# Fannovel16/stylish-tts

Hardware: AMD Instinct MI355X
Metric: utterances_per_sec (higher is better)
Workload: dtype f32

## Files before the change

include/stylish_hip.h:

```cpp
#ifndef STYLISH_HIP_H_
#define STYLISH_HIP_H_

#include <stddef.h>
#include <stdint.h>

#ifdef __cplusplus
extern "C" {
#endif

typedef struct stts_ctx stts_ctx;

typedef struct stts_model_dims {
  int32_t n_fft, win_length, hop_length, sample_rate;
  int32_t style_dim, inter_dim;
  int32_t dec_hidden, dec_residual;
  int32_t gen_input, gen_hidden, gen_inter, gen_io_kernel;
  int32_t tokens, te_hidden, te_filter, te_heads, te_layers, te_kernel;
  int32_t style_layers;
  int32_t dur_layers, dur_classes, dur_max;
  int32_t pe_inter;
} stts_model_dims;

const char* stts_last_error(void);
int stts_version(void);
// ... 77 lines not shown
} stts_cfm_dims;
int stts_cfm_finalize(stts_ctx* ctx, const stts_cfm_dims* dims);
size_t stts_cfm_workspace_bytes(const stts_ctx* ctx, int64_t rows, int n_utt);
int stts_cfm_estimator(stts_ctx* ctx, void* stream, int n_utt, const int32_t* seg_off_host, const int32_t* seg_off_dev, const float* x, int ld_x,
                       const float* asr, int ld_asr, const float* f0, const float* n_curve, const int32_t* curve_off_host,
                       const int32_t* curve_off_dev, const float* spk_emb, const float* t, const float* sine_noise, float* out, int ld_out,
                       void* workspace, size_t workspace_bytes);

int stts_to_time_major(void* stream, const float* x_bct, int B, int C, int T, float* y, int ldy);
int stts_to_channel_major(void* stream, const float* x, int ldx, int B, int C, int T, float* y_bct);

int stts_conv_stft_transform(stts_ctx* ctx, void* stream, int n_utt, const int32_t* frame_off_host, const int32_t* frame_off_dev,
                             const float* wave, int hop, float* mag, float* x, float* y, int ld);
int stts_conv_stft_inverse(stts_ctx* ctx, void* stream, int n_utt, const int32_t* frame_off_host, const int32_t* frame_off_dev,
                           const float* mag, const float* x, const float* y, int ld, int hop, float* wave_out, void* ws, size_t ws_bytes);

int stts_profile_begin(void);
int stts_profile_end(void* stream, int* launches, double* total_ms, double* total_flops);
int stts_profile_report(void* stream, char* json, size_t json_capacity);

int stts_op_mrf_block(stts_ctx* ctx, void* stream, const char* prefix, int n_utt, const int32_t* seg_off_host,
                      const int32_t* seg_off_dev, const float* x, int ldx, int channels, int kernel, const float* style, float* y,
                      int ldy, void* ws, size_t ws_bytes);

#ifdef STTS_TEST_OPS
int stts_op_conv1d(void* stream, int n_utt, const int32_t* seg_off_host, const int32_t* seg_off_dev, const float* x, int ldx, int cin,
                   const float* w_host, const float* bias_host, int cout, int k, int dil, int act, float* y, int ldy, int force_tile, int precision);
int stts_op_adain_block(stts_ctx* ctx, void* stream, const char* prefix, int n_utt, const int32_t* seg_off_host,
                        const int32_t* seg_off_dev, const float* x, int ldx, int cin, int cout, const float* style, float* y, int ldy,
                        void* ws, size_t ws_bytes);
int stts_op_attention(void* stream, int n_utt, const int32_t* q_off_host, const int32_t* q_off_dev, const int32_t* k_off_host,
                      const int32_t* k_off_dev, const float* q, const float* k, const float* v, float* o, int heads, int kc,
                      const int32_t* band_centre, int window, int kernel);
int stts_bench_gemm(void* stream, int n_utt, int rows_per_utt, int cin, int cout, int k, int tile, int iters, double* avg_ms, int tune);
#endif

#ifdef __cplusplus
}
#endif
#endif
```

stylish_tts_amd/_lib.py:

```python
from __future__ import annotations

import ctypes as C
import os

_HERE = os.path.dirname(os.path.abspath(__file__))
LIB_PATH = os.path.abspath(os.environ["STTS_LIB"]) if os.environ.get("STTS_LIB") else os.path.join(_HERE, "libstylish_hip.so")


class ModelDims(C.Structure):
    _fields_ = [(n, C.c_int32) for n in (
        "n_fft", "win_length", "hop_length", "sample_rate",
        "style_dim", "inter_dim",
        "dec_hidden", "dec_residual",
        "gen_input", "gen_hidden", "gen_inter", "gen_io_kernel",
        "tokens", "te_hidden", "te_filter", "te_heads", "te_layers", "te_kernel",
        "style_layers",
        "dur_layers", "dur_classes", "dur_max",
        "pe_inter",
    )]


class CfmDims(C.Structure):
    _fields_ = [(n, C.c_int32) for n in ("feat_dim", "asr_dim", "spk_dim", "hidden_dim", "emb_dim", "depth", "enc_blocks", "dec_blocks",
                                         "prev_depth", "post_depth", "head_dim")]
# ... 30 lines not shown
    "stts_har_ld": (_I, [_P]),
    "stts_decoder_forward": (_I, [_P, _P, _I, _P, _P, _P, _I, _P, _P, _P, _P, _I, _P, _SZ]),
    "stts_prior_flow_forward": (_I, [_P, _P, _I, _P, _P, _P, _I, _P, _P, _P, _I, _P, _P, _P, _SZ]),
    "stts_harmonic_stft": (_I, [_P, _P, _I, _P, _P, _P, _P, _P, _I, _P, _P, _P, _I, _P, _SZ]),
    "stts_vocoder_forward": (_I, [_P, _P, _I, _P, _P, _P, _I, _P, _P, _P, _I, _P, _P, _P, _I, _P, _SZ]),
    "stts_frame_path": (_I, [_P, _P, _I, _P, _P, _P, _I, _P, _P, _P, _P, _P, _P, _I, _P, _P, _SZ, _I]),
    "stts_frame_offsets": (_I, [_P, _P, _I, _P, _P, _P, _P, _P, _P]),
    "stts_phoneme_workspace_bytes": (_SZ, [_P, _I64, _I64, _I]),
    "stts_text_encoder_forward": (_I, [_P, _P, _I, _I, _P, _P, _P, _P, _I, _P, _P, _SZ]),
    "stts_text_style_forward": (_I, [_P, _P, _I, _I, _P, _P, _P, _I, _P, _P, _SZ]),
    "stts_duration_forward": (_I, [_P, _P, _I, _P, _P, _P, _P, _P, _P, _P, _P, _P, _SZ]),
    "stts_pitch_energy_forward": (_I, [_P, _P, _I, _P, _P, _P, _P, _P, _P, _I, _P, _P, _P, _P, _P, _P, _SZ, _I]),
    "stts_duration_decode": (_I, [_P, _P, _I, _I, _P]),
    "stts_duration_to_alignment": (_I, [_P, _P, _I, _I, _P]),
    "stts_length_regulate": (_I, [_P, _P, _I, _P, _P, _P, _I64, _I, _P, _I, _I, _P, _I, _P]),
    "stts_set_precision": (_I, [_P, _I]),
    "stts_upsample4": (_I, [_P, _P, _I, _P, _P, _P, _P, _P]),
    "stts_euler_step": (_I, [_P, _P, _P, C.c_float, C.c_int64]),
    "stts_cfm_finalize": (_I, [_P, _P]),
    "stts_cfm_workspace_bytes": (_SZ, [_P, _I64, _I]),
    "stts_cfm_estimator": (_I, [_P, _P, _I, _P, _P, _P, _I, _P, _I, _P, _P, _P, _P, _P, _P, _P, _P, _I, _P, _SZ]),
    "stts_to_time_major": (_I, [_P, _P, _I, _I, _I, _P, _I]),
    "stts_to_channel_major": (_I, [_P, _P, _I, _I, _I, _I, _P]),
    "stts_conv_stft_transform": (_I, [_P, _P, _I, _P, _P, _P, _I, _P, _P, _P, _I]),
    "stts_conv_stft_inverse": (_I, [_P, _P, _I, _P, _P, _P, _P, _P, _I, _I, _P, _P, _SZ]),
    "stts_profile_begin": (_I, []),
    "stts_profile_end": (_I, [_P, C.POINTER(_I), C.POINTER(C.c_double), C.POINTER(C.c_double)]),
    "stts_profile_report": (_I, [_P, C.c_char_p, _SZ]),
    "stts_op_mrf_block": (_I, [_P, _P, C.c_char_p, _I, _P, _P, _P, _I, _I, _I, _P, _P, _I, _P, _SZ]),
}
TEST_SIGNATURES = {
    "stts_bench_gemm": (_I, [_P, _I, _I, _I, _I, _I, _I, _I, C.POINTER(C.c_double), _I]),
    "stts_op_conv1d": (_I, [_P, _I, _P, _P, _P, _I, _I, _P, _P, _I, _I, _I, _I, _P, _I, _I, _I]),
    "stts_op_adain_block": (_I, [_P, _P, C.c_char_p, _I, _P, _P, _P, _I, _I, _I, _P, _P, _I, _P, _SZ]),
    "stts_op_attention": (_I, [_P, _I, _P, _P, _P, _P, _P, _P, _P, _P, _I, _I, _P, _I, _I]),
}

_lib = None


def load() -> C.CDLL:
    global _lib
    if _lib is not None:
        return _lib
    if not os.path.exists(LIB_PATH):
        raise RuntimeError(
            f"{LIB_PATH} not found: build it with `python -c 'import __graft_entry__ as g; g.build()'` "
            "(hipcc --offload-arch=gfx950).  There is no CPU fallback."
        )
    try:
        import torch
    except ImportError:
        pass
    lib = C.CDLL(LIB_PATH)
    for name, (res, args) in SIGNATURES.items():
        fn = getattr(lib, name)
        fn.restype = res
        fn.argtypes = args
    for name, (res, args) in TEST_SIGNATURES.items():
        fn = getattr(lib, name, None)
        if fn is not None:
            fn.restype = res
            fn.argtypes = args
    _lib = lib
    return lib

# ... 5 lines not shown
```

stylish_tts_amd/csrc/gemm.hip.h:

```cpp
#pragma once
#include <type_traits>
#include <mutex>
#include <map>
#include <hip/hip_ext.h>
#include <cmath>
#include <algorithm>
#include <vector>

#include "common.h"

namespace stts {

using f32x16 = __attribute__((ext_vector_type(16))) float;
using f32x4 = __attribute__((ext_vector_type(4))) float;

enum Act { ACT_NONE = 0, ACT_SILU = 1, ACT_GELU = 2, ACT_RELU = 3, ACT_LRELU = 4 };
enum Epi {
  EPI_STORE = 0,
  EPI_GATE = 1,
  EPI_SPLIT_ACC = 2,
  EPI_COUPLE = 3,
  EPI_PRIOR = 4,
};

// ... 83 lines not shown
  u32x2 r;
  if constexpr (PREC == PREC_BF16) {
    typedef __bf16 b2 __attribute__((ext_vector_type(2)));
    typedef float f2 __attribute__((ext_vector_type(2)));
    const f2 lo = {v.x, v.y}, hi = {v.z, v.w};
    r.x = __builtin_bit_cast(unsigned, __builtin_convertvector(lo, b2));
    r.y = __builtin_bit_cast(unsigned, __builtin_convertvector(hi, b2));
  } else {
    typedef _Float16 h2 __attribute__((ext_vector_type(2)));
    typedef float f2 __attribute__((ext_vector_type(2)));
    const f2 lo = {v.x, v.y}, hi = {v.z, v.w};
    r.x = __builtin_bit_cast(unsigned, __builtin_convertvector(lo, h2));
    r.y = __builtin_bit_cast(unsigned, __builtin_convertvector(hi, h2));
  }
  return r;
}
__device__ __forceinline__ void split3_bf16(const f32x4 v, u32x2& p0, u32x2& p1, u32x2& p2) {
  typedef __bf16 b2 __attribute__((ext_vector_type(2)));
  typedef float f2 __attribute__((ext_vector_type(2)));
  auto pk = [](float a, float b) { const f2 t = {a, b}; return __builtin_bit_cast(unsigned, __builtin_convertvector(t, b2)); };
  auto lo = [](unsigned u) { return __uint_as_float(u << 16); };
  auto hi = [](unsigned u) { return __uint_as_float(u & 0xffff0000u); };
  p0.x = pk(v.x, v.y); p0.y = pk(v.z, v.w);
  const float r0 = v.x - lo(p0.x), r1 = v.y - hi(p0.x), r2 = v.z - lo(p0.y), r3 = v.w - hi(p0.y);
  p1.x = pk(r0, r1); p1.y = pk(r2, r3);
  p2.x = pk(r0 - lo(p1.x), r1 - hi(p1.x)); p2.y = pk(r2 - lo(p1.y), r3 - hi(p1.y));
}
template <int PREC>
__device__ __forceinline__ f32x16 mfma16(const f32x4 a, const f32x4 b, const f32x16 c) {
  if constexpr (PREC == PREC_BF16 || PREC == PREC_X3) return __builtin_amdgcn_mfma_f32_32x32x16_bf16(__builtin_bit_cast(bf16x8, a), __builtin_bit_cast(bf16x8, b), c, 0, 0, 0);
  else return __builtin_amdgcn_mfma_f32_32x32x16_f16(__builtin_bit_cast(f16x8, a), __builtin_bit_cast(f16x8, b), c, 0, 0, 0);
}

template <int BM, int BN, int WARPS_M, int WARPS_N, int EPI, int KSPLIT = 1, bool GLDS = false, int PREC = PREC_F32, int XAFF = 0, bool MSEG = true,
          bool X16 = false>
__global__ void __launch_bounds__(WARPS_M* WARPS_N * 64 * KSPLIT) conv_gemm_f32(const GemmArgs a) {
  static_assert(!(XAFF && GLDS), "the input affine lives on the register staging path");
  static_assert(!X16 || (PREC != PREC_F32 && !XAFF && EPI == EPI_STORE), "16-bit activation rows: 16-bit operand modes, store epilogue");
  constexpr int NT = WARPS_M * WARPS_N * 64 * KSPLIT;
  constexpr bool B16 = PREC != PREC_F32;
  constexpr bool X3 = PREC == PREC_X3;
  constexpr int NPL = X3 ? 3 : 1;
  static_assert(!X3 || !GLDS || X16, "split fp32: fp32 activation rows are split on the register staging path; LDS-DMA needs pre-split planes");
  static_assert(!(B16 && GLDS) || X16, "LDS-DMA staging of 16-bit operands needs 16-bit activation rows (nothing converts on the way)");
  static_assert(KSPLIT == 1 || KSPLIT == 2, "KSPLIT");
  constexpr int WR = BN / WARPS_N, WC = BM / WARPS_M;
  constexpr int TR = WR / 32, TC = WC / 32;
  constexpr int XL = X16 ? (BN * 4 * NPL + NT - 1) / NT : BN * 8 / NT;
  constexpr int WL = B16 ? (BM * 4 * NPL + NT - 1) / NT : BM * 8 / NT;
  static_assert(WR % 32 == 0 && WC % 32 == 0, "wave tile must be a multiple of 32x32");
  static_assert((X16 || (BN * 8) % NT == 0) && (B16 || (BM * 8) % NT == 0), "tile loads must divide over the block");
  static_assert(EPI == EPI_STORE || EPI == EPI_SPLIT_ACC || TC % 2 == 0, "paired epilogues need an even TC");
  constexpr int NSTAGE = (B16 && GLDS) ? (X3 ? 3 : ((BM + BN) <= 256 ? 8 : 3)) : 2;
  constexpr int SLOTS = X3 ? 12 : ((B16 && KSPLIT == 1) ? 4 : 8);
  constexpr int PLANE = (BN + BM) * 4;
  constexpr int STG16 = PLANE * NPL;
  __shared__ f32x4 lds[NSTAGE * (BN + BM) * SLOTS];

  int bx = blockIdx.x, by = blockIdx.y, bz = blockIdx.z;
  {
    unsigned gy = gridDim.y;
    if (a.capacity) {
      const int lane_ = threadIdx.x & 63;
      int tot = 0;
      for (int u0 = 0; u0 < a.n_utt; u0 += 64) {
        const int u = u0 + lane_;
        tot += u < a.n_utt ? (a.seg_off[u + 1] - a.seg_off[u] + BN - 1) / BN : 0;
      }
#pragma unroll
      for (int o = 32; o > 0; o >>= 1) tot += __shfl_xor(tot, o, 64);
      gy = (unsigned)__builtin_amdgcn_readfirstlane(tot);
      if ((unsigned)by >= gy) return;
    }
    const unsigned gx = gridDim.x, nwg = gx * gy * gridDim.z;
    const unsigned orig = bx + gx * (by + gy * bz);
    const unsigned q = nwg >> 3, r = nwg & 7, xcd = orig & 7;
    const unsigned id = (xcd < r ? xcd * (q + 1) : r * (q + 1) + (xcd - r) * q) + (orig >> 3);
    bx = id % gx;
    by = (id / gx) % gy;
    bz = id / (gx * gy);
  }
  const int ksplit = a.ksplit > 1 ? a.ksplit : 1;
  int utt, ks;
  if (a.compact) {
    ks = bz;
    const int t = by + a.tile0, lane_ = threadIdx.x & 63;
    utt = a.n_utt - 1;
    int base = 0, local = 0;
    bool done = false;
    if (a.uniform_len > 0) {
      const int tpu = (a.uniform_len + BN - 1) / BN;
      utt = t / tpu;
      local = t - utt * tpu;
      done = utt < a.n_utt;
    }
    for (int u0 = 0; u0 < a.n_utt && !done && a.uniform_len <= 0; u0 += 64) {
      const int u = u0 + lane_;
      const int tiles = u < a.n_utt ? (a.seg_off[u + 1] - a.seg_off[u] + BN - 1) / BN : 0;
      int incl = tiles;
#pragma unroll
      for (int d = 1; d < 64; d <<= 1) {
        const int v = __shfl_up(incl, d, 64);
        if (lane_ >= d) incl += v;
      }
      const int excl = incl - tiles;
      const unsigned long long hit = __ballot(t >= base + excl && t < base + incl);
      if (hit) {
        const int src = __ffsll((long long)hit) - 1;
        utt = u0 + src;
        local = t - base - __shfl(excl, src, 64);
        done = true;
      }
      base += __shfl(incl, 63, 64);
    }
    if (!done) return;
    utt = __builtin_amdgcn_readfirstlane(utt);
    by = __builtin_amdgcn_readfirstlane(local);
  } else {
    utt = bz / ksplit;
    ks = bz % ksplit;
  }
  const int lo = a.uniform_len > 0 ? a.uniform_lo0 + utt * a.uniform_len : a.seg_off[utt];
  const int hi = a.uniform_len > 0 ? lo + a.uniform_len : a.seg_off[utt + 1];
  const int row0 = lo + by * BN;
  if (row0 >= hi) return;
  const int m0 = bx * BM;
  const int tid = threadIdx.x, lane = tid & 63;
#ifdef STTS_GEMM_TRACE
  const unsigned dbg_blk = blockIdx.x + gridDim.x * (blockIdx.y + gridDim.y * blockIdx.z);
  auto stamp = [&](int i) { if (a.dbg && tid == 0) a.dbg[8 * (long)dbg_blk + i] = wall_clock64(); };
  const long long dbg_c0 = clock64();
  if (a.dbg && tid == 0) { a.dbg[8 * (long)dbg_blk + 5] = __builtin_amdgcn_s_getreg(0xF804); a.dbg[8 * (long)dbg_blk + 6] = __builtin_amdgcn_s_getreg(0xF814); }
  auto stamp_end = [&]() { stamp(3); if (a.dbg && tid == 0) a.dbg[8 * (long)dbg_blk + 7] = clock64() - dbg_c0; };
  auto ablate = [&](int bit) { return (a.tune & bit) != 0; };
#else
  auto stamp = [&](int) {};
  auto stamp_end = [&]() {};
  auto ablate = [](int) { return false; };
#endif
  stamp(0);
  const int kg = (tid >> 6) / (WARPS_M * WARPS_N), wid = (tid >> 6) % (WARPS_M * WARPS_N);
  const int wn = wid / WARPS_M, wm = wid % WARPS_M;
  (void)kg;

  f32x16 acc[TR][TC];
#pragma unroll
  for (int i = 0; i < TR; ++i)
#pragma unroll
    for (int j = 0; j < TC; ++j)
#pragma unroll
      for (int r = 0; r < 16; ++r) acc[i][j][r] = 0.0f;

  int s = 0, tap = 0, chunk = 0;
  auto xbase = [&](const GemmSeg& g) {
// ... 812 lines not shown
  for (int i = 0; i < a.nseg; ++i) k += (double)a.seg[i].kreal * a.seg[i].ntaps;
  return 2.0 * (double)a.rows_total * (double)a.wrows * k;
}

#define STTS_LAUNCH_TIMED(kernel, grid, block, st, e0, e1, ...)                                   \
  do {                                                                                            \
    if (e0) hipExtLaunchKernelGGL(kernel, grid, block, 0, st, e0, e1, 0, __VA_ARGS__);            \
    else hipLaunchKernelGGL(kernel, grid, block, 0, st, __VA_ARGS__);                             \
  } while (0)

#define STTS_LAUNCH_PROF(name, bytes, kernel, grid, block, st, ...)                                \
  do {                                                                                            \
    stts::GemmProfiler& _p = stts::gemm_profiler();                                               \
    if (_p.on) {                                                                                  \
      hipEvent_t _e0 = _p.next(), _e1 = _p.next();                                                \
      _p.add(name, 1, 0.0, 0.0, (double)(bytes));                                                 \
      hipExtLaunchKernelGGL(kernel, grid, block, 0, st, _e0, _e1, 0, __VA_ARGS__);                \
    } else {                                                                                      \
      hipLaunchKernelGGL(kernel, grid, block, 0, st, __VA_ARGS__);                                \
    }                                                                                             \
  } while (0)

inline bool gemm16_eligible(const GemmArgs& a, int epi, int npad);
inline long gemm16_tiles(const GemmArgs& a, int npad, int n_utt);
inline bool gemm16_will_run(const GemmArgs& a, int epi, int npad, int n_utt);
template <int ABL>
inline int launch_conv_gemm16(hipStream_t st, const GemmArgs& a, int npad, int n_utt);

void gemm_dispatch_f32(hipStream_t st, const GemmArgs& as, int tile, int epi, int npad, int n_utt, int max_rows, hipEvent_t e0, hipEvent_t e1);
void gemm_dispatch_bf16(hipStream_t st, const GemmArgs& as, int tile, int epi, int npad, int n_utt, int max_rows, hipEvent_t e0, hipEvent_t e1);
void gemm_dispatch_f16(hipStream_t st, const GemmArgs& as, int tile, int epi, int npad, int n_utt, int max_rows, hipEvent_t e0, hipEvent_t e1);
void gemm_dispatch_x3(hipStream_t st, const GemmArgs& as, int tile, int epi, int npad, int n_utt, int max_rows, hipEvent_t e0, hipEvent_t e1);
int launch_conv_gemm16_main(hipStream_t st, const GemmArgs& a, int npad, int n_utt);

#ifndef STTS_GEMM_NO_LAUNCHER
template <int BM, int BN, int WM, int WN, int KS = 1, bool GL = false, int PR = PREC_F32>
inline void launch_cfg(hipStream_t st, const GemmArgs& a, int epi, int npad, int n_utt, int max_rows, hipEvent_t e0 = nullptr, hipEvent_t e1 = nullptr) {
  dim3 grid(npad / BM, ceil_div(max_rows, BN), n_utt * (a.ksplit > 1 ? a.ksplit : 1)), block(WM * WN * 64 * KS);
  if (a.compact) grid = dim3(npad / BM, a.tiles_y, a.ksplit > 1 ? a.ksplit : 1);
  if constexpr (GL && PR != PREC_F32) {
    if (a.nseg == 1) STTS_LAUNCH_TIMED((conv_gemm_f32<BM, BN, WM, WN, EPI_STORE, KS, true, PR, false, false, true>), grid, block, st, e0, e1, a);
    else STTS_LAUNCH_TIMED((conv_gemm_f32<BM, BN, WM, WN, EPI_STORE, KS, true, PR, false, true, true>), grid, block, st, e0, e1, a);
    return;
  } else
  switch (epi) {
    case EPI_STORE:
      if constexpr (!GL && PR != PREC_F32 && KS == 1) {
        if (a.x16) {
          if (a.nseg == 1) STTS_LAUNCH_TIMED((conv_gemm_f32<BM, BN, WM, WN, EPI_STORE, KS, GL, PR, false, false, true>), grid, block, st, e0, e1, a);
          else STTS_LAUNCH_TIMED((conv_gemm_f32<BM, BN, WM, WN, EPI_STORE, KS, GL, PR, false, true, true>), grid, block, st, e0, e1, a);
          break;
        }
      }
      if constexpr (!GL) {
        if (a.xaff) {
          if (a.nseg == 1) STTS_LAUNCH_TIMED((conv_gemm_f32<BM, BN, WM, WN, EPI_STORE, KS, GL, PR, 1, false>), grid, block, st, e0, e1, a);
          else STTS_LAUNCH_TIMED((conv_gemm_f32<BM, BN, WM, WN, EPI_STORE, KS, GL, PR, 1, true>), grid, block, st, e0, e1, a);
          break;
        }
        if (a.nseg == 1) {
          STTS_LAUNCH_TIMED((conv_gemm_f32<BM, BN, WM, WN, EPI_STORE, KS, GL, PR, false, false>), grid, block, st, e0, e1, a);
          break;
        }
      }
      STTS_LAUNCH_TIMED((conv_gemm_f32<BM, BN, WM, WN, EPI_STORE, KS, GL, PR>), grid, block, st, e0, e1, a);
      break;
// ... 45 lines not shown
      break;
    case 16:
      if constexpr (PR != PREC_F32) launch_cfg<256, 256, 4, 2, 1, true, PR>(st, as, epi, npad, n_utt, max_rows, e0, e1);
      break;
    case 17:
      if constexpr (PR != PREC_F32) launch_cfg<128, 256, 4, 2, 1, true, PR>(st, as, epi, npad, n_utt, max_rows, e0, e1);
      break;
    case 18:
      if constexpr (PR != PREC_F32) launch_cfg<128, 128, 4, 2, 1, true, PR>(st, as, epi, npad, n_utt, max_rows, e0, e1);
      break;
    case 11:
      if constexpr (PR == PREC_F32) launch_cfg<128, 128, 4, 2, 1, true>(st, as, epi, npad, n_utt, max_rows, e0, e1);
      break;
    case 13:
      if constexpr (PR == PREC_F32) launch_cfg<128, 64, 4, 2, 1, true>(st, as, epi, npad, n_utt, max_rows, e0, e1);
      break;
    default: launch_cfg<128, 32, 2, 1, 1, false, PR>(st, as, epi, npad, n_utt, max_rows, e0, e1); break;
  }
}
inline void gemm_dispatch_tile_x3(hipStream_t st, const GemmArgs& as, int tile, int epi, int npad, int n_utt, int max_rows, hipEvent_t e0, hipEvent_t e1) {
  switch (tile) {
    case 2: launch_cfg_x3<128, 64, 2, 2>(st, as, epi, npad, n_utt, max_rows, e0, e1); break;
    case 4: launch_cfg_x3<128, 32, 4, 1>(st, as, epi, npad, n_utt, max_rows, e0, e1); break;
    case 5: launch_cfg_x3<128, 128, 4, 2>(st, as, epi, npad, n_utt, max_rows, e0, e1); break;
    case 6: launch_cfg_x3<128, 64, 4, 2>(st, as, epi, npad, n_utt, max_rows, e0, e1); break;
    case 8: launch_cfg_x3<128, 128, 4, 2, 2>(st, as, epi, npad, n_utt, max_rows, e0, e1); break;
    case 20: launch_cfg_x3<128, 128, 2, 2>(st, as, epi, npad, n_utt, max_rows, e0, e1); break;
    case 21: launch_cfg_x3<128, 128, 2, 2, 2>(st, as, epi, npad, n_utt, max_rows, e0, e1); break;
    case 22: launch_cfg_x3<128, 256, 2, 4>(st, as, epi, npad, n_utt, max_rows, e0, e1); break;
    case 25: launch_cfg_x3<128, 128, 4, 2, 1, 1>(st, as, epi, npad, n_utt, max_rows, e0, e1); break;
    case 26: launch_cfg_x3<128, 64, 4, 2, 1, 1>(st, as, epi, npad, n_utt, max_rows, e0, e1); break;
    case 27: launch_cfg_x3<128, 128, 4, 2, 1, 2>(st, as, epi, npad, n_utt, max_rows, e0, e1); break;
    case 28: launch_cfg_x3<128, 64, 4, 2, 1, 2>(st, as, epi, npad, n_utt, max_rows, e0, e1); break;
    default: launch_cfg_x3<128, 32, 2, 1>(st, as, epi, npad, n_utt, max_rows, e0, e1); break;
  }
}
inline bool x3_enabled() {
  static const bool on = !(getenv("STTS_NO_X3") && atoi(getenv("STTS_NO_X3")) != 0);
  return on;
}

inline int launch_conv_gemm(hipStream_t st, const GemmArgs& a, int epi, int npad, int n_utt, int max_rows, int force_tile = 0) {
  STTS_CHECK(npad % 128 == 0, "conv_gemm: padded cout %d not a multiple of 128", npad);
  for (int i = 0; i < a.nseg; ++i) {
    STTS_CHECK(a.seg[i].kc % 32 == 0 && a.seg[i].ldx % 4 == 0 && a.seg[i].xcol0 % 4 == 0, "conv_gemm: segment %d misaligned (kc %d ldx %d xcol0 %d)", i,
               a.seg[i].kc, a.seg[i].ldx, a.seg[i].xcol0);
  }
  if (a.x16 && a.prec != PREC_F32)
    for (int i = 0; i < a.nseg; ++i)
      STTS_CHECK(a.seg[i].ldx % 8 == 0 && a.seg[i].xcol0 % 8 == 0, "conv_gemm: 16-bit activation rows need ldx / xcol0 multiples of 8 (segment %d)", i);
  if (force_tile == 19 || (force_tile == 0 && gemm16_will_run(a, epi, npad, n_utt))) {
    if (gemm16_eligible(a, epi, npad)) return launch_conv_gemm16_main(st, a, npad, n_utt);
  }
  STTS_CHECK(!a.stat_part, "conv_gemm: output statistics (stat_part) exist only in conv_gemm16_kernel's epilogue: ask gemm16_will_run first");
  STTS_CHECK(force_tile != 19, "conv_gemm: tile 19 (conv_gemm16_kernel) needs 16-bit activation rows, a store epilogue, channels in multiples of 64 and cout padded to 256");
  constexpr int kCUs = 256;
  const int mt = npad / 128;
  auto row_tiles = [&](int bn) -> long {
    if (!a.seg_host) return (long)n_utt * ceil_div(max_rows, bn);
    long t = 0;
    for (int u = 0; u < n_utt; ++u) t += ceil_div(a.seg_host[u + 1] - a.seg_host[u], bn);
    return t;
  };
  int iters = 0;
  for (int i = 0; i < a.nseg; ++i) iters += a.seg[i].ntaps * (a.seg[i].kc / 32);
  const bool splittable = force_tile == 0 && epi == EPI_STORE && !a.sumsq_part && a.Y && !a.Y16;
// ... 7 lines not shown
    Plan p;
    const long rt = row_tiles(bn), blocks = rt * mt;
    const long whole = blocks / kCUs;
    p.full_rt = rt;
    p.cost = std::ceil((double)blocks / kCUs);
    static const bool x3_rem = getenv("STTS_X3_REM") && atoi(getenv("STTS_X3_REM")) != 0;
    if ((!x3 || x3_rem) && splittable && a.seg_host && !a.capacity && whole >= 1 && blocks % kCUs != 0) {
      const long full_rt = whole * kCUs / mt, rem_blocks = (rt - full_rt) * mt;
      const int ksp = (int)std::min<long>(8, std::min<long>(iters / 4, kCUs / std::max<long>(rem_blocks, 1)));
      if (ksp >= 2 && full_rt > 0) {
        const double hybrid = (double)(full_rt * mt) / kCUs + std::max((double)rem_blocks / kCUs, 1.0 / ksp) * 1.15 + 0.1;
        if (hybrid < p.cost) {
          p.full_rt = full_rt;
          p.rem_rt = rt - full_rt;
          p.rem_ksp = ksp;
          p.cost = hybrid;
        }
      }
    }
    p.cost *= bn * penalty;
    return p;
  };
  const long blocks128 = mt * row_tiles(128);
  x3 = a.prec == PREC_F32 && x3_enabled() && (epi == EPI_STORE || epi == EPI_PRIOR);
  for (int i = 0; i < a.nseg; ++i) x3 = x3 && a.seg[i].W16 != nullptr && a.seg[i].w16_plane > 0 && 6 * a.seg[i].w16_plane + 2L * 128 * a.seg[i].ntaps * a.seg[i].kc < (1L << 32);
  if (a.x16 && a.prec == PREC_F32) {
    STTS_CHECK(x3 && epi == EPI_STORE && !a.xaff && !a.sumsq_part, "conv_gemm: pre-split activation planes need the split-fp32 store contraction");
    for (int i = 0; i < a.nseg; ++i) STTS_CHECK(a.seg[i].x_plane > 0 && a.seg[i].ldx % 8 == 0 && a.seg[i].xcol0 % 8 == 0, "conv_gemm: pre-split activation planes: segment %d misaligned", i);
  }
  if (force_tile >= 100) {
    x3 = false;
    force_tile -= 100;
  }
  if (force_tile != 0 && !((force_tile >= 2 && force_tile <= 6) || force_tile == 8 || (force_tile >= 20 && force_tile <= 22) || (a.x16 && force_tile >= 25 && force_tile <= 28))) x3 = false;
  int tile = force_tile;
  const bool paired = epi != EPI_STORE && epi != EPI_SPLIT_ACC;
  Plan plan;
  if (tile == 0) {
    if (blocks128 < 24) tile = paired ? 3 : 4;
    else if (paired) tile = 2;
    else {
      const Plan p5 = plan_for(128, 1.0), p6 = plan_for(64, 1.03);
      tile = p5.cost <= p6.cost ? 5 : 6;
      if (x3 && iters <= 24 && !a.xaff) tile = 6;
      plan = tile == 5 ? p5 : p6;
      if (tile == 5 && blocks128 <= kCUs && a.prec == PREC_F32 && !x3) tile = 8;
    }
  }
  if (force_tile == 0 && a.prec != PREC_F32 && a.x16 && epi == EPI_STORE) {
    const long rt256 = row_tiles(256);
    if (npad % 256 == 0 && iters >= 128 && rt256 * (npad / 256) >= 3 * kCUs / 2) tile = 14;
    else if (rt256 * (npad / 128) >= 3 * kCUs / 2) tile = 15;
    if (tile == 14 || tile == 15) plan = Plan();
    if (const char* e = getenv("STTS_TILE16")) {
      tile = atoi(e);
      plan = Plan();
    }
  }
  STTS_CHECK(!(a.x16 && (tile == 8 || tile == 11 || tile == 13 || a.xaff)), "conv_gemm: 16-bit activation rows need a plain register-staged tile");
  STTS_CHECK(!((tile == 14 || tile == 15) && (a.prec == PREC_F32 || epi != EPI_STORE)), "conv_gemm: tiles 14 / 15 are for 16-bit operand store launches");
  STTS_CHECK(!((tile >= 16 && tile <= 18) && (a.prec == PREC_F32 || epi != EPI_STORE || !a.x16)), "conv_gemm: tiles 16 - 18 are for 16-bit activation rows, store epilogue");
  STTS_CHECK((tile != 14 && tile != 16) || npad % 256 == 0, "conv_gemm: tiles 14 / 16 need cout padded to 256");
  if (x3 && !a.x16 && force_tile == 0 && (tile == 5 || tile == 6)) {
    static const int x3_tile = getenv("STTS_X3_TILE") ? atoi(getenv("STTS_X3_TILE")) : 0;
    if (x3_tile == 5 || x3_tile == 6 || x3_tile == 22) {
      tile = x3_tile;
      plan = Plan();
    }
  }
  const long blocks22 = row_tiles(256) * mt;
  const bool fills22 = blocks22 >= 640 || (blocks22 >= 440 && (blocks22 % kCUs == 0 || blocks22 % kCUs >= kCUs * 4 / 5));
  if (x3 && !a.x16 && force_tile == 0 && (tile == 5 || tile == 6) && fills22 && !getenv("STTS_X3_TILE")) {
    tile = 22;
    plan = Plan();
  }
  STTS_CHECK(!(tile >= 20 && tile <= 28) || x3, "conv_gemm: tiles 20 - 28 exist for the split-fp32 contractions only");
  if (x3 && a.x16) {
    static const int gl_env = getenv("STTS_X3P_GLDS") ? atoi(getenv("STTS_X3P_GLDS")) : 1;
    if (tile < 25) tile = (tile == 5 || tile == 8 || tile == 20 || tile == 21 || tile == 22) ? (gl_env ? 27 : 25) : (gl_env ? 28 : 26);
    plan = Plan();
  }
  STTS_CHECK(!(tile >= 25 && tile <= 28) || (x3 && a.x16), "conv_gemm: tiles 25 - 28 read pre-split activation planes");
  const int bn = ((tile >= 14 && tile <= 17) || tile == 22) ? 256 : (tile == 5 || tile == 8 || tile == 11 || tile == 18 || tile == 20 || tile == 21 || tile == 25 || tile == 27) ? 128 : ((tile == 3 || tile == 4) ? 32 : 64);
  if (plan.full_rt == 0 && plan.rem_rt == 0) plan.full_rt = row_tiles(bn);
  if (tile == 8 || tile == 21) {
    plan.full_rt = row_tiles(bn);
    plan.rem_rt = 0;
  }
  GemmArgs as = a;
  as.n_utt = n_utt;
  if (!as.zeros) as.zeros = zero_page();
  as.compact = a.seg_host != nullptr;
  int main_ksp = 1;
  if (splittable && tile != 8 && tile != 21 && tile < 25 && plan.rem_rt == 0) {
    const long blocks = plan.full_rt * mt;
    static const int min_it_env = getenv("STTS_SPLITK_MIN_ITERS") ? std::max(1, atoi(getenv("STTS_SPLITK_MIN_ITERS"))) : 0;
    const int min_it = min_it_env ? min_it_env : (blocks >= 128 ? 8 : 4);
    main_ksp = (int)std::min<long>(8, std::min<long>(iters / min_it, ((a.prec == PREC_F32 && !x3) ? 512 : 255) / std::max<long>(blocks, 1)));
    if (main_ksp < 2) main_ksp = 1;
  }
  float* part = nullptr;
  if (main_ksp > 1 || plan.rem_rt > 0) {
    part = splitk_scratch(st, (size_t)std::max(main_ksp, plan.rem_ksp) * a.rows_total * npad * sizeof(float));
    if (!part) {
      main_ksp = 1;
      plan.full_rt += plan.rem_rt;
      plan.rem_rt = 0;
    }
  }
  if (a.prec != PREC_F32) {
    for (int i = 0; i < a.nseg; ++i) STTS_CHECK(a.seg[i].W16 != nullptr, "conv_gemm: 16-bit operand mode without 16-bit weights (segment %d)", i);
    STTS_CHECK(tile != 11 && tile != 13, "conv_gemm: LDS-DMA tiles are fp32 only");
  }
  GemmProfiler& prof = gemm_profiler();
  const double flops = gemm_algorithmic_flops(a);
  const long all_rt = plan.full_rt + plan.rem_rt;
// ... 65 lines not shown
```

stylish_tts_amd/csrc/gemm_tu_x3.hip:

```cpp
#define STTS_GEMM_TU_FORM 3
#include "gemm.hip.h"
```

Baseline: 2522.

## Add multi-stage pipelined split-fp32 GEMM kernel for pre-split activation planes

Adds a dedicated conv-GEMM kernel for the split-fp32 (x3) path with pre-split 16-bit activation planes. It uses a 3- or 4-stage global-to-LDS async load pipeline with explicit vmcnt waits and optional wave priority boosting around the MFMA block. The tile lookup is factored into a shared helper. By default the dispatcher now routes x3/x16 store launches without Y16 to the new tiles 29/30, trading code size and LDS pressure for better latency hiding.

New measurement: 2535, median of 6. Within noise of the previous version (+0.5%).

```diff
diff --git a/include/stylish_hip.h b/include/stylish_hip.h
--- a/include/stylish_hip.h
+++ b/include/stylish_hip.h
@@ -133,6 +133,8 @@
 int stts_op_attention(void* stream, int n_utt, const int32_t* q_off_host, const int32_t* q_off_dev, const int32_t* k_off_host,
                       const int32_t* k_off_dev, const float* q, const float* k, const float* v, float* o, int heads, int kc,
                       const int32_t* band_centre, int window, int kernel);
+int stts_op_conv1d_x3p(void* stream, int n_utt, const int32_t* seg_off_host, const int32_t* seg_off_dev, int capacity, const float* x, int ldx,
+                       int cin, const float* w_host, int cout, int k, float* y, int ldy, int tile, int nseg);
 int stts_bench_gemm(void* stream, int n_utt, int rows_per_utt, int cin, int cout, int k, int tile, int iters, double* avg_ms, int tune);
 #endif
 
diff --git a/stylish_tts_amd/_lib.py b/stylish_tts_amd/_lib.py
--- a/stylish_tts_amd/_lib.py
+++ b/stylish_tts_amd/_lib.py
@@ -86,6 +86,7 @@
 TEST_SIGNATURES = {
     "stts_bench_gemm": (_I, [_P, _I, _I, _I, _I, _I, _I, _I, C.POINTER(C.c_double), _I]),
     "stts_op_conv1d": (_I, [_P, _I, _P, _P, _P, _I, _I, _P, _P, _I, _I, _I, _I, _P, _I, _I, _I]),
+    "stts_op_conv1d_x3p": (_I, [_P, _I, _P, _P, _I, _P, _I, _I, _P, _I, _I, _P, _I, _I, _I]),
     "stts_op_adain_block": (_I, [_P, _P, C.c_char_p, _I, _P, _P, _P, _I, _I, _I, _P, _P, _I, _P, _SZ]),
     "stts_op_attention": (_I, [_P, _I, _P, _P, _P, _P, _P, _P, _P, _P, _I, _I, _P, _I, _I]),
 }
diff --git a/stylish_tts_amd/csrc/gemm.hip.h b/stylish_tts_amd/csrc/gemm.hip.h
--- a/stylish_tts_amd/csrc/gemm.hip.h
+++ b/stylish_tts_amd/csrc/gemm.hip.h
@@ -139,6 +139,74 @@
   else return __builtin_amdgcn_mfma_f32_32x32x16_f16(__builtin_bit_cast(f16x8, a), __builtin_bit_cast(f16x8, b), c, 0, 0, 0);
 }
 
+template <int BN>
+__device__ __forceinline__ bool gemm_tile_lookup(const GemmArgs& a, int ksplit, int& bx, int& by, int& utt, int& ks) {
+  bx = blockIdx.x;
+  by = blockIdx.y;
+  int bz = blockIdx.z;
+  {
+    unsigned gy = gridDim.y;
+    if (a.capacity) {
+      const int lane_ = threadIdx.x & 63;
+      int tot = 0;
+      for (int u0 = 0; u0 < a.n_utt; u0 += 64) {
+        const int u = u0 + lane_;
+        tot += u < a.n_utt ? (a.seg_off[u + 1] - a.seg_off[u] + BN - 1) / BN : 0;
+      }
+#pragma unroll
+      for (int o = 32; o > 0; o >>= 1) tot += __shfl_xor(tot, o, 64);
+      gy = (unsigned)__builtin_amdgcn_readfirstlane(tot);
+      if ((unsigned)by >= gy) return false;
+    }
+    const unsigned gx = gridDim.x, nwg = gx * gy * gridDim.z;
+    const unsigned orig = bx + gx * (by + gy * bz);
+    const unsigned q = nwg >> 3, r = nwg & 7, xcd = orig & 7;
+    const unsigned id = (xcd < r ? xcd * (q + 1) : r * (q + 1) + (xcd - r) * q) + (orig >> 3);
+    bx = id % gx;
+    by = (id / gx) % gy;
+    bz = id / (gx * gy);
+  }
+  if (a.compact) {
+    ks = bz;
+    const int t = by + a.tile0, lane_ = threadIdx.x & 63;
+    utt = a.n_utt - 1;
+    int base = 0, local = 0;
+    bool done = false;
+    if (a.uniform_len > 0) {
+      const int tpu = (a.uniform_len + BN - 1) / BN;
+      utt = t / tpu;
+      local = t - utt * tpu;
+      done = utt < a.n_utt;
+    }
+    for (int u0 = 0; u0 < a.n_utt && !done && a.uniform_len <= 0; u0 += 64) {
+      const int u = u0 + lane_;
+      const int tiles = u < a.n_utt ? (a.seg_off[u + 1] - a.seg_off[u] + BN - 1) / BN : 0;
+      int incl = tiles;
+#pragma unroll
+      for (int d = 1; d < 64; d <<= 1) {
+        const int v = __shfl_up(incl, d, 64);
+        if (lane_ >= d) incl += v;
+      }
+      const int excl = incl - tiles;
+      const unsigned long long hit = __ballot(t >= base + excl && t < base + incl);
+      if (hit) {
+        const int src = __ffsll((long long)hit) - 1;
+        utt = u0 + src;
+        local = t - base - __shfl(excl, src, 64);
+        done = true;
+      }
+      base += __shfl(incl, 63, 64);
+    }
+    if (!done) return false;
+    utt = __builtin_amdgcn_readfirstlane(utt);
+    by = __builtin_amdgcn_readfirstlane(local);
+  } else {
+    utt = bz / ksplit;
+    ks = bz % ksplit;
+  }
+  return true;
+}
+
 template <int BM, int BN, int WARPS_M, int WARPS_N, int EPI, int KSPLIT = 1, bool GLDS = false, int PREC = PREC_F32, int XAFF = 0, bool MSEG = true,
           bool X16 = false>
 __global__ void __launch_bounds__(WARPS_M* WARPS_N * 64 * KSPLIT) conv_gemm_f32(const GemmArgs a) {
@@ -164,69 +232,9 @@
   constexpr int STG16 = PLANE * NPL;
   __shared__ f32x4 lds[NSTAGE * (BN + BM) * SLOTS];
 
-  int bx = blockIdx.x, by = blockIdx.y, bz = blockIdx.z;
-  {
-    unsigned gy = gridDim.y;
-    if (a.capacity) {
-      const int lane_ = threadIdx.x & 63;
-      int tot = 0;
-      for (int u0 = 0; u0 < a.n_utt; u0 += 64) {
-        const int u = u0 + lane_;
-        tot += u < a.n_utt ? (a.seg_off[u + 1] - a.seg_off[u] + BN - 1) / BN : 0;
-      }
-#pragma unroll
-      for (int o = 32; o > 0; o >>= 1) tot += __shfl_xor(tot, o, 64);
-      gy = (unsigned)__builtin_amdgcn_readfirstlane(tot);
-      if ((unsigned)by >= gy) return;
-    }
-    const unsigned gx = gridDim.x, nwg = gx * gy * gridDim.z;
-    const unsigned orig = bx + gx * (by + gy * bz);
-    const unsigned q = nwg >> 3, r = nwg & 7, xcd = orig & 7;
-    const unsigned id = (xcd < r ? xcd * (q + 1) : r * (q + 1) + (xcd - r) * q) + (orig >> 3);
-    bx = id % gx;
-    by = (id / gx) % gy;
-    bz = id / (gx * gy);
-  }
+  int bx, by, utt, ks;
   const int ksplit = a.ksplit > 1 ? a.ksplit : 1;
-  int utt, ks;
-  if (a.compact) {
-    ks = bz;
-    const int t = by + a.tile0, lane_ = threadIdx.x & 63;
-    utt = a.n_utt - 1;
-    int base = 0, local = 0;
-    bool done = false;
-    if (a.uniform_len > 0) {
-      const int tpu = (a.uniform_len + BN - 1) / BN;
-      utt = t / tpu;
-      local = t - utt * tpu;
-      done = utt < a.n_utt;
-    }
-    for (int u0 = 0; u0 < a.n_utt && !done && a.uniform_len <= 0; u0 += 64) {
-      const int u = u0 + lane_;
-      const int tiles = u < a.n_utt ? (a.seg_off[u + 1] - a.seg_off[u] + BN - 1) / BN : 0;
-      int incl = tiles;
-#pragma unroll
-      for (int d = 1; d < 64; d <<= 1) {
-        const int v = __shfl_up(incl, d, 64);
-        if (lane_ >= d) incl += v;
-      }
-      const int excl = incl - tiles;
-      const unsigned long long hit = __ballot(t >= base + excl && t < base + incl);
-      if (hit) {
-        const int src = __ffsll((long long)hit) - 1;
-        utt = u0 + src;
-        local = t - base - __shfl(excl, src, 64);
-        done = true;
-      }
-      base += __shfl(incl, 63, 64);
-    }
-    if (!done) return;
-    utt = __builtin_amdgcn_readfirstlane(utt);
-    by = __builtin_amdgcn_readfirstlane(local);
-  } else {
-    utt = bz / ksplit;
-    ks = bz % ksplit;
-  }
+  if (!gemm_tile_lookup<BN>(a, ksplit, bx, by, utt, ks)) return;
   const int lo = a.uniform_len > 0 ? a.uniform_lo0 + utt * a.uniform_len : a.seg_off[utt];
   const int hi = a.uniform_len > 0 ? lo + a.uniform_len : a.seg_off[utt + 1];
   const int row0 = lo + by * BN;
@@ -1105,6 +1113,7 @@
 void gemm_dispatch_f16(hipStream_t st, const GemmArgs& as, int tile, int epi, int npad, int n_utt, int max_rows, hipEvent_t e0, hipEvent_t e1);
 void gemm_dispatch_x3(hipStream_t st, const GemmArgs& as, int tile, int epi, int npad, int n_utt, int max_rows, hipEvent_t e0, hipEvent_t e1);
 int launch_conv_gemm16_main(hipStream_t st, const GemmArgs& a, int npad, int n_utt);
+void launch_conv_gemm_x3p(hipStream_t st, const GemmArgs& a, int tile, int npad, int n_utt, int max_rows, hipEvent_t e0, hipEvent_t e1);
 
 #ifndef STTS_GEMM_NO_LAUNCHER
 template <int BM, int BN, int WM, int WN, int KS = 1, bool GL = false, int PR = PREC_F32>
@@ -1216,6 +1225,8 @@
     case 26: launch_cfg_x3<128, 64, 4, 2, 1, 1>(st, as, epi, npad, n_utt, max_rows, e0, e1); break;
     case 27: launch_cfg_x3<128, 128, 4, 2, 1, 2>(st, as, epi, npad, n_utt, max_rows, e0, e1); break;
     case 28: launch_cfg_x3<128, 64, 4, 2, 1, 2>(st, as, epi, npad, n_utt, max_rows, e0, e1); break;
+    case 29:
+    case 30: launch_conv_gemm_x3p(st, as, tile, npad, n_utt, max_rows, e0, e1); break;
     default: launch_cfg_x3<128, 32, 2, 1>(st, as, epi, npad, n_utt, max_rows, e0, e1); break;
   }
 }
@@ -1289,7 +1300,7 @@
     x3 = false;
     force_tile -= 100;
   }
-  if (force_tile != 0 && !((force_tile >= 2 && force_tile <= 6) || force_tile == 8 || (force_tile >= 20 && force_tile <= 22) || (a.x16 && force_tile >= 25 && force_tile <= 28))) x3 = false;
+  if (force_tile != 0 && !((force_tile >= 2 && force_tile <= 6) || force_tile == 8 || (force_tile >= 20 && force_tile <= 22) || (a.x16 && force_tile >= 25 && force_tile <= 30))) x3 = false;
   int tile = force_tile;
   const bool paired = epi != EPI_STORE && epi != EPI_SPLIT_ACC;
   Plan plan;
@@ -1331,14 +1342,19 @@
     tile = 22;
     plan = Plan();
   }
-  STTS_CHECK(!(tile >= 20 && tile <= 28) || x3, "conv_gemm: tiles 20 - 28 exist for the split-fp32 contractions only");
+  STTS_CHECK(!(tile >= 20 && tile <= 30) || x3, "conv_gemm: tiles 20 - 30 exist for the split-fp32 contractions only");
   if (x3 && a.x16) {
+    static const int pipe_env = getenv("STTS_X3P_PIPE") ? atoi(getenv("STTS_X3P_PIPE")) : 1;
     static const int gl_env = getenv("STTS_X3P_GLDS") ? atoi(getenv("STTS_X3P_GLDS")) : 1;
-    if (tile < 25) tile = (tile == 5 || tile == 8 || tile == 20 || tile == 21 || tile == 22) ? (gl_env ? 27 : 25) : (gl_env ? 28 : 26);
+    const bool t128 = tile == 5 || tile == 8 || tile == 20 || tile == 21 || tile == 22;
+    if (tile < 25) tile = (pipe_env && !a.Y16) ? (t128 ? 29 : 30) : t128 ? (gl_env ? 27 : 25) : (gl_env ? 28 : 26);
     plan = Plan();
   }
-  STTS_CHECK(!(tile >= 25 && tile <= 28) || (x3 && a.x16), "conv_gemm: tiles 25 - 28 read pre-split activation planes");
-  const int bn = ((tile >= 14 && tile <= 17) || tile == 22) ? 256 : (tile == 5 || tile == 8 || tile == 11 || tile == 18 || tile == 20 || tile == 21 || tile == 25 || tile == 27) ? 128 : ((tile == 3 || tile == 4) ? 32 : 64);
+  STTS_CHECK(!(tile >= 25 && tile <= 30) || (x3 && a.x16), "conv_gemm: tiles 25 - 30 read pre-split activation planes");
+  STTS_CHECK(!(tile >= 29 && tile <= 30) || (!a.Y16 && !a.sumsq_part && epi == EPI_STORE), "conv_gemm: tiles 29 / 30 have the plain store epilogue only");
+  const int bn = ((tile >= 14 && tile <= 17) || tile == 22) ? 256
+                 : (tile == 5 || tile == 8 || tile == 11 || tile == 18 || tile == 20 || tile == 21 || tile == 25 || tile == 27 || tile == 29) ? 128
+                 : ((tile == 3 || tile == 4) ? 32 : 64);
   if (plan.full_rt == 0 && plan.rem_rt == 0) plan.full_rt = row_tiles(bn);
   if (tile == 8 || tile == 21) {
     plan.full_rt = row_tiles(bn);
diff --git a/stylish_tts_amd/csrc/gemm_tu_x3.hip b/stylish_tts_amd/csrc/gemm_tu_x3.hip
--- a/stylish_tts_amd/csrc/gemm_tu_x3.hip
+++ b/stylish_tts_amd/csrc/gemm_tu_x3.hip
@@ -1,2 +1,3 @@
 #define STTS_GEMM_TU_FORM 3
 #include "gemm.hip.h"
+#include "gemm_x3.hip.h"
diff --git a/stylish_tts_amd/csrc/gemm_x3.hip.h b/stylish_tts_amd/csrc/gemm_x3.hip.h
--- /dev/null
+++ b/stylish_tts_amd/csrc/gemm_x3.hip.h
@@ -0,0 +1,223 @@
+#pragma once
+#include "gemm.hip.h"
+
+namespace stts {
+
+template <int N>
+__device__ __forceinline__ void x3_wait_vm() {
+  static_assert(N >= 0 && N <= 63, "vmcnt immediate");
+  asm volatile("" ::: "memory");
+  __builtin_amdgcn_s_waitcnt((N & 15) | (7 << 4) | (15 << 8) | ((N >> 4) << 14));
+  asm volatile("" ::: "memory");
+}
+
+template <int BM, int BN, int NSTAGE, bool MSEG, bool PRIO>
+__global__ void __launch_bounds__(512) conv_gemm_x3_kernel(const GemmArgs a) {
+  constexpr int WARPS_M = 4, WARPS_N = 2, NW = WARPS_M * WARPS_N;
+  constexpr int WR = BN / WARPS_N, WC = BM / WARPS_M, TR = WR / 32, TC = WC / 32;
+  static_assert(WR % 32 == 0 && WC % 32 == 0 && BN % 16 == 0, "wave tile must be a multiple of 32 x 32");
+  constexpr int PLANE = (BN + BM) * 4;
+  constexpr int STG = 3 * PLANE;
+  constexpr int NI1 = (BN + BM) / 16, NI = 3 * NI1;
+  constexpr int PER = (NI + NW - 1) / NW;
+  static_assert(NSTAGE >= 3 && NSTAGE <= 4, "the tail waits below are written for three or four stages");
+  static_assert((NSTAGE - 2) * PER <= 63, "vmcnt immediate");
+  static_assert(NSTAGE * STG * 16 <= 160 * 1024, "LDS");
+  __shared__ f32x4 lds[NSTAGE * STG];
+
+  int bx, by, utt, ks;
+  if (!gemm_tile_lookup<BN>(a, 1, bx, by, utt, ks)) return;
+  (void)ks;
+  const int lo = a.uniform_len > 0 ? a.uniform_lo0 + utt * a.uniform_len : a.seg_off[utt];
+  const int hi = a.uniform_len > 0 ? lo + a.uniform_len : a.seg_off[utt + 1];
+  const int row0 = lo + by * BN;
+  if (row0 >= hi) return;
+  const int m0 = bx * BM;
+  const int tid = threadIdx.x, lane = tid & 63;
+  const int wv = tid >> 6;
+  const int wn = __builtin_amdgcn_readfirstlane(wv) / WARPS_M, wm = __builtin_amdgcn_readfirstlane(wv) % WARPS_M;
+  const int l31 = lane & 31, lh = lane >> 5;
+  const int len = hi - lo, rel0 = row0 - lo;
+
+  f32x16 acc[TR][TC];
+#pragma unroll
+  for (int i = 0; i < TR; ++i)
+#pragma unroll
+    for (int j = 0; j < TC; ++j)
+#pragma unroll
+      for (int r = 0; r < 16; ++r) acc[i][j][r] = 0.0f;
+
+  int s = 0, tap = 0, chunk = 0;
+  const unsigned short* gX = reinterpret_cast<const unsigned short*>(a.seg[0].X) + a.seg[0].xcol0;
+  const unsigned short* gW = a.seg[0].W16 + (long)utt * a.seg[0].w_utt_stride + (long)m0 * a.seg[0].ntaps * a.seg[0].kc;
+  int g_ldx = a.seg[0].ldx, g_kc = a.seg[0].kc, g_ntaps = a.seg[0].ntaps, g_dil = a.seg[0].dil, g_pad = a.seg[0].pad;
+  long g_wplane = a.seg[0].w16_plane, g_xplane = a.seg[0].x_plane;
+  int total = a.seg[0].ntaps * (a.seg[0].kc / 32);
+  if constexpr (MSEG) {
+    if (a.nseg > 1) total += a.seg[1].ntaps * (a.seg[1].kc / 32);
+    if (a.nseg > 2) total += a.seg[2].ntaps * (a.seg[2].kc / 32);
+  }
+
+  auto issue = [&](int b) {
+    const int shift = (tap - g_pad) * g_dil;
+    const char* xb = reinterpret_cast<const char*>(gX + (long)lo * g_ldx + chunk * 32);
+    const char* wb = reinterpret_cast<const char*>(gW + tap * g_kc + chunk * 32);
+    const int wrow = g_ntaps * g_kc;
+#pragma unroll
+    for (int q = 0; q < PER; ++q) {
+      const int instq = min(wv + q * NW, NI - 1);
+      const int pl = instq / NI1, inst = instq % NI1;
+      const int trow = inst * 16 + (lane >> 2);
+      const int n = trow - BN, sslot = (lane & 3) ^ ((trow >> 2) & 3);
+      const int rel = rel0 + trow + shift;
+      const bool ok = rel >= 0 && rel < len;
+      const char* xsrc = ok ? xb + pl * g_xplane * 2 + (unsigned)((rel * g_ldx + sslot * 8) * 2) : reinterpret_cast<const char*>(a.zeros);
+      const char* wsrc = wb + pl * g_wplane * 2 + (unsigned)((n * wrow + sslot * 8) * 2);
+      const char* src = inst < BN / 16 ? xsrc : wsrc;
+      __builtin_amdgcn_global_load_lds((const __attribute__((address_space(1))) void*)src,
+                                       (__attribute__((address_space(3))) void*)(lds + b * STG + pl * PLANE + inst * 64), 16, 0, 0);
+    }
+    const int w1 = tap + 1 >= g_ntaps, wk = (chunk + 1) * 32 >= g_kc;
+    const bool wrapt = (w1 & wk) != 0;
+    tap = w1 ? 0 : tap + 1;
+    chunk = wrapt ? 0 : chunk + w1;
+    if constexpr (MSEG) {
+      if (wrapt && s + 1 < a.nseg) {
+        ++s;
+        const GemmSeg& n = s == 1 ? a.seg[1] : a.seg[2];
+        gX = reinterpret_cast<const unsigned short*>(n.X) + n.xcol0;
+        gW = n.W16 + (long)utt * n.w_utt_stride + (long)m0 * n.ntaps * n.kc;
+        g_ldx = n.ldx; g_kc = n.kc; g_ntaps = n.ntaps; g_dil = n.dil; g_pad = n.pad;
+        g_wplane = n.w16_plane; g_xplane = n.x_plane;
+      }
+    }
+  };
+  auto wait_ahead = [&](int ahead) {
+    if (NSTAGE == 4 && ahead >= 2) x3_wait_vm<(NSTAGE == 4 ? 2 * PER : 0)>();
+    else if (ahead >= 1) x3_wait_vm<PER>();
+    else x3_wait_vm<0>();
+  };
+  auto barrier = [&]() {
+    asm volatile("s_waitcnt lgkmcnt(0)" ::: "memory");
+    __builtin_amdgcn_s_barrier();
+    asm volatile("" ::: "memory");
+  };
+  auto mma_half = [&](int b, int kk) {
+    const f32x4* Xs = lds + b * STG;
+    const f32x4* Ws = Xs + BN * 4;
+    const int slot = 2 * kk + lh;
+    f32x4 xa[TR][3], wb[TC][3];
+#pragma unroll
+    for (int i = 0; i < TR; ++i) {
+      const int r = wn * WR + i * 32 + l31;
+      const int o = r * 4 + (slot ^ ((r >> 2) & 3));
+#pragma unroll
+      for (int p = 0; p < 3; ++p) xa[i][p] = Xs[o + p * PLANE];
+    }
+#pragma unroll
+    for (int j = 0; j < TC; ++j) {
+      const int c = wm * WC + j * 32 + l31;
+      const int o = c * 4 + (slot ^ ((c >> 2) & 3));
+#pragma unroll
+      for (int p = 0; p < 3; ++p) wb[j][p] = Ws[o + p * PLANE];
+    }
+    if constexpr (PRIO) __builtin_amdgcn_s_setprio(1);
+#pragma unroll
+    for (int i = 0; i < TR; ++i)
+#pragma unroll
+      for (int j = 0; j < TC; ++j) {
+        acc[i][j] = mfma16<PREC_X3>(xa[i][2], wb[j][0], acc[i][j]);
+        acc[i][j] = mfma16<PREC_X3>(xa[i][0], wb[j][2], acc[i][j]);
+        acc[i][j] = mfma16<PREC_X3>(xa[i][1], wb[j][1], acc[i][j]);
+        acc[i][j] = mfma16<PREC_X3>(xa[i][1], wb[j][0], acc[i][j]);
+        acc[i][j] = mfma16<PREC_X3>(xa[i][0], wb[j][1], acc[i][j]);
+        acc[i][j] = mfma16<PREC_X3>(xa[i][0], wb[j][0], acc[i][j]);
+      }
+    if constexpr (PRIO) __builtin_amdgcn_s_setprio(0);
+  };
+
+  const int npro = min(total, NSTAGE - 1);
+#pragma unroll
+  for (int q = 0; q < NSTAGE - 1; ++q)
+    if (q < npro) issue(q);
+  wait_ahead(npro - 1);
+  barrier();
+  int it = 0, cur = 0, nxt = NSTAGE - 1;
+  for (; it < total - (NSTAGE - 1); ++it) {
+    issue(nxt);
+    mma_half(cur, 0);
+    mma_half(cur, 1);
+    x3_wait_vm<(NSTAGE - 2) * PER>();
+    barrier();
+    cur = cur == NSTAGE - 1 ? 0 : cur + 1;
+    nxt = nxt == NSTAGE - 1 ? 0 : nxt + 1;
+  }
+  for (; it < total; ++it) {
+    mma_half(cur, 0);
+    mma_half(cur, 1);
+    if (it + 1 < total) {
+      wait_ahead(total - it - 2);
+      barrier();
+    }
+    cur = cur == NSTAGE - 1 ? 0 : cur + 1;
+  }
+
+  const int nvalid = hi - row0;
+  const bool hasR = a.R != nullptr, hasY = a.Y != nullptr;
+  const int act = a.act;
+  const float alpha = a.alpha;
+  float* const Yb = hasY ? a.Y + (long)row0 * a.ldy + a.ycol0 + m0 : nullptr;
+  const float* const Rb = hasR ? a.R + (long)row0 * a.ldr + a.rcol0 + m0 : nullptr;
+  const int rlane = wn * WR + 4 * lh, clane = wm * WC + l31;
+  unsigned oy = (unsigned)(rlane * a.ldy + clane), orr = (unsigned)(rlane * a.ldr + clane);
+  const unsigned sy1 = (unsigned)a.ldy, sy5 = 5u * sy1, sr1 = (unsigned)a.ldr, sr5 = 5u * sr1;
+  float bv[TC];
+  bool nok[TC];
+#pragma unroll
+  for (int j = 0; j < TC; ++j) {
+    const int n = m0 + clane + j * 32;
+    bv[j] = a.bias ? a.bias[n] : 0.0f;
+    nok[j] = n < a.N;
+  }
+#pragma unroll
+  for (int i = 0; i < TR; ++i) {
+#pragma unroll
+    for (int r = 0; r < 16; ++r) {
+      const int dr = i * 32 + (r & 3) + 8 * (r >> 2);
+      const bool rok = rlane + dr < nvalid;
+#pragma unroll
+      for (int j = 0; j < TC; ++j) {
+        float v = act_apply(acc[i][j][r] + bv[j], act);
+        if (rok && nok[j]) {
+          if (hasR) v += Rb[orr + j * 32];
+          v *= alpha;
+          if (hasY) Yb[oy + j * 32] = v;
+        }
+      }
+      const bool big = (r & 3) == 3;
+      oy += big ? sy5 : sy1;
+      orr += big ? sr5 : sr1;
+    }
+    __builtin_amdgcn_sched_barrier(0);
+  }
+}
+
+template <int BM, int BN, int NSTAGE>
+inline void launch_x3p_cfg(hipStream_t st, const GemmArgs& a, int npad, int n_utt, int max_rows, hipEvent_t e0, hipEvent_t e1) {
+  dim3 grid(npad / BM, ceil_div(max_rows, BN), n_utt), block(512);
+  if (a.compact) grid = dim3(npad / BM, a.tiles_y, 1);
+  static const bool prio = !(getenv("STTS_X3P_PRIO") && atoi(getenv("STTS_X3P_PRIO")) == 0);
+  if (a.nseg == 1) {
+    if (prio) STTS_LAUNCH_TIMED((conv_gemm_x3_kernel<BM, BN, NSTAGE, false, true>), grid, block, st, e0, e1, a);
+    else STTS_LAUNCH_TIMED((conv_gemm_x3_kernel<BM, BN, NSTAGE, false, false>), grid, block, st, e0, e1, a);
+  } else {
+    if (prio) STTS_LAUNCH_TIMED((conv_gemm_x3_kernel<BM, BN, NSTAGE, true, true>), grid, block, st, e0, e1, a);
+    else STTS_LAUNCH_TIMED((conv_gemm_x3_kernel<BM, BN, NSTAGE, true, false>), grid, block, st, e0, e1, a);
+  }
+}
+void launch_conv_gemm_x3p(hipStream_t st, const GemmArgs& a, int tile, int npad, int n_utt, int max_rows, hipEvent_t e0, hipEvent_t e1) {
+  if (tile == 29) launch_x3p_cfg<128, 128, 3>(st, a, npad, n_utt, max_rows, e0, e1);
+  else launch_x3p_cfg<128, 64, 4>(st, a, npad, n_utt, max_rows, e0, e1);
+}
+
+}
```
